# ayildiri/polymer-chemprop

Measured on AMD Instinct MI355X. Metric: edges/sec MPN forward, batch=64 polymer graphs, depth=3 hidden=300, higher is better.
Workload: dtype fp32; 1 GPU; MPNEncoder.forward on synthetic polymer batches of 64 graphs (avg E=6164 directed edges), depth=3, hidden=300, 8 resident batches cycled per rank; global_batch=64, depth=3, hidden=300, parallelism=dp1 (independent graphs, no collective in the forward), streams=3

## Files before the change

### polymer-chemprop_amd/csrc/fused_mp.hpp

```cpp
#pragma once
#include "gemm_x6.hpp"
#include "kernels.hpp"
#include "wdmpnn.h"

namespace wd {


constexpr int BLK_BONDS = 128, BLK_ATOMS = 64;
constexpr int BLK_MOLS = 64;
constexpr int ELLW = 8;
static_assert(ELLW % 4 == 0, "ELL rows of whole 4-byte index words and float4 weight groups");

struct EllRow {
    uint32_t ix[ELLW / 4];
    float w[ELLW];
};
__device__ __forceinline__ EllRow ell_zero() {
    EllRow e;
    for (int k = 0; k < ELLW / 4; ++k) e.ix[k] = 0;
    for (int k = 0; k < ELLW; ++k) e.w[k] = 0.f;
    return e;
}
__device__ __forceinline__ EllRow ell_load(const uint8_t *idx, const float *coef, size_t row) {
    EllRow e;
// ... 52 lines not shown
    const uint8_t *ain; int ain_g;
    uint8_t *aout;
    uint8_t *apairs;
};

template <int BM, int AACT>
struct H2Prod {
    static constexpr int U = BM / 64;
    static constexpr int SETS = 3;
    __amdgpu_buffer_rsrc_t rs;
    int off[U];
    uint32_t grow[U];
    int r0, u, live16;
    float slope, scale, pd;
    uint64_t seed;
    uint32_t layer;
    uint32_t wv;
    u32x4 v[SETS][U][2];
    __device__ __forceinline__ void init() { scale = h2_scale(wave_max_u32(wv)); }
    __device__ __forceinline__ H2Prod(const MpLayerP &P, int rs0, int rn, uint32_t words) {
        const int t = threadIdx.x & 255;
        r0 = t >> 2; u = t & 3;
        rs = __builtin_amdgcn_make_buffer_rsrc(const_cast<float *>(P.zin + (size_t)rs0 * P.ldz), 0,
                                               rn > 0 ? ((rn - 1) * P.ldz + P.kp) * 4 : 0, 0x00020000);
#pragma unroll
        for (int i = 0; i < U; ++i) {
            const int r = r0 + 64 * i;
            grow[i] = r < rn ? rs0 + r : 0;
            off[i] = (r * P.ldz + 8 * u) * 4;
        }
        live16 = (rn + 15) & ~15;
        slope = AACT == ACT_PRELU ? P.slope[0] : 0.f;
        wv = words;
        scale = 1.f;
        pd = P.p_drop_in;
        seed = P.seed;
        layer = P.layer - 1;
    }
    template <typename S>
    __device__ __forceinline__ void load(S, int kc) {
#pragma unroll
        for (int i = 0; i < U; ++i)
#pragma unroll
            for (int h = 0; h < 2; ++h)
                v[S::value][i][h] = __builtin_bit_cast(u32x4, __builtin_amdgcn_raw_buffer_load_b128(rs, off[i] + 128 * kc + 16 * h, 0, 0));
    }
    template <typename S>
    __device__ __forceinline__ void store(S, int kc, uint8_t *st) {
#pragma unroll
        for (int i = 0; i < U; ++i)
#pragma unroll
            for (int h = 0; h < 2; ++h) asm volatile("" ::"v"(v[S::value][i][h]));
#pragma unroll
        for (int i = 0; i < U; ++i) {
            const int r = r0 + 64 * i;
            if (r >= live16) continue;
            float x[8];
#pragma unroll
            for (int h = 0; h < 2; ++h) {
                const u32x4 a = v[S::value][i][h];
                x[4 * h] = __uint_as_float(a.x); x[4 * h + 1] = __uint_as_float(a.y);
                x[4 * h + 2] = __uint_as_float(a.z); x[4 * h + 3] = __uint_as_float(a.w);
            }
#pragma unroll
            for (int q = 0; q < 8; ++q) x[q] = act_fwd(AACT, x[q], slope);
            if (pd > 0.f)
#pragma unroll
                for (int q = 0; q < 8; ++q) x[q] *= dropout_scale(seed, layer, grow[i], 32 * kc + 8 * u + q, pd);
            uint32_t hh[4], ll[4];
#pragma unroll
            for (int q = 0; q < 4; ++q) split_h2(x[2 * q], x[2 * q + 1], scale, hh[q], ll[q]);
            uint8_t *d = st + x6_slot(r, u);
            *reinterpret_cast<u32x4 *>(d) = u32x4{hh[0], hh[1], hh[2], hh[3]};
            *reinterpret_cast<u32x4 *>(d + BM * 64) = u32x4{ll[0], ll[1], ll[2], ll[3]};
        }
    }
};

#ifndef WD_ZWT
#define WD_ZWT 0
#endif

constexpr int MP_THREADS = 512;

template <int BN, int NT, bool LAST, bool ATOM = false, bool POUT = false>
struct MpEpilogue {
    static constexpr int BM = BLK_BONDS, LDC = BN + 4;
    static constexpr int UPR = BN / 8, UNITS = BM * UPR, UPT = (UNITS + NT - 1) / NT;
    static constexpr int AUNITS = BLK_ATOMS * UPR, AUPT = (AUNITS + NT - 1) / NT;
    static constexpr int LDS_FLOATS = (BM + BLK_ATOMS) * LDC;
    static constexpr int YPT = ATOM ? AUPT : UPT;
    EllRow aell[AUPT];
    EllRow gell[ATOM && LAST ? AUPT : 1];
    int32_t rv[ATOM ? 1 : UPT];
    uint32_t sa[ATOM ? 1 : UPT];

    __device__ __forceinline__ void prefetch(const MpLayerP &P, const BlockRow &B) {
        const int tid = threadIdx.x;
#pragma unroll
        for (int i = 0; i < AUPT; ++i) {
            const int v = tid + NT * i;
            const bool ok = v < AUNITS && v / UPR < B.an;
            aell[i] = ell_zero();
            if (ok) aell[i] = ATOM ? ell_load(P.mell_idx, P.mell_coef, (size_t)B.as + v / UPR)
                                   : ell_load(P.aell_idx, P.aell_coef, (size_t)B.as + v / UPR);
            if constexpr (ATOM && LAST) {
                gell[i] = ell_zero();
                if (ok) gell[i] = ell_load(P.aell_idx, P.aell_coef, (size_t)B.as + v / UPR);
            }
        }
        if constexpr (!ATOM)
#pragma unroll
            for (int i = 0; i < UPT; ++i) {
                const int v = tid + NT * i, lr = v / UPR;
                rv[i] = 0;
                sa[i] = 0;
                if (v < UNITS && lr < B.bn) {
                    rv[i] = P.rev[B.bs + lr];
                    sa[i] = P.src_blk[B.bs + lr];
                }
            }
    }

    static constexpr int PRE_ELL = BLK_ATOMS * (int)sizeof(EllRow);
    static constexpr int PRE_BYTES = PRE_ELL * (ATOM && LAST ? 2 : 1) + (ATOM ? 0 : BM * 8);
    __device__ __forceinline__ void fill_pre(const MpLayerP &P, const BlockRow &B, uint8_t *pre) {
        const int t = threadIdx.x - MP_THREADS / 2;
        if (t < BLK_ATOMS) {
            EllRow e = ell_zero();
            if (t < B.an) e = ATOM ? ell_load(P.mell_idx, P.mell_coef, (size_t)B.as + t)
                                   : ell_load(P.aell_idx, P.aell_coef, (size_t)B.as + t);
            reinterpret_cast<EllRow *>(pre)[t] = e;
            if constexpr (ATOM && LAST) {
                EllRow f = ell_zero();
                if (t < B.an) f = ell_load(P.aell_idx, P.aell_coef, (size_t)B.as + t);
                reinterpret_cast<EllRow *>(pre + PRE_ELL)[t] = f;
            }
        }
        if constexpr (!ATOM)
            if (t < BM) {
                int2 q = make_int2(0, 0);
                if (t < B.bn) q = make_int2(P.rev[B.bs + t], (int)P.src_blk[B.bs + t]);
                reinterpret_cast<int2 *>(pre + PRE_ELL)[t] = q;
            }
    }
    __device__ __forceinline__ void take_pre(const BlockRow &B, const uint8_t *pre) {
        const int tid = threadIdx.x;
#pragma unroll
        for (int i = 0; i < AUPT; ++i) {
            const int v = tid + NT * i, la = min(v / UPR, BLK_ATOMS - 1);
            aell[i] = reinterpret_cast<const EllRow *>(pre)[la];
            if constexpr (ATOM && LAST) gell[i] = reinterpret_cast<const EllRow *>(pre + PRE_ELL)[la];
        }
        if constexpr (!ATOM)
#pragma unroll
            for (int i = 0; i < UPT; ++i) {
                const int v = tid + NT * i, lr = min(v / UPR, BM - 1);
                const int2 q = reinterpret_cast<const int2 *>(pre + PRE_ELL)[lr];
                rv[i] = q.x;
                sa[i] = (uint32_t)q.y;
            }
    }

    __device__ __forceinline__ void row_sum(const int32_t *ptr, const int32_t *idx, const float *coef, int row, int base,
                                            const EllRow &E, int c, const float *T, float4 &s0, float4 &s1) {
        s0 = s1 = f4zero();
#pragma unroll
        for (int k = 0; k < ELLW; ++k)
            if (E.w[k] != 0.f) lds_term<LDC>(T, ell_idx(E, k), c, E.w[k], s0, s1);
        if (ell_more(E))
            for (int q = ptr[row] + ELLW; q < ptr[row + 1]; ++q) {
                const int li = idx[q] - base;
                if (li >= 0) lds_term<LDC>(T, li, c, coef ? coef[q] : 1.0f, s0, s1);
            }
    }
    __device__ __forceinline__ void atom_sum(const MpLayerP &P, const BlockRow &B, const EllRow &E, int la, int c,
                                             const float *T, float4 &s0, float4 &s1) {
        row_sum(P.aptr, P.aidx, P.acoef, B.as + la, ATOM ? B.as : B.bs, E, c, T, s0, s1);
    }

    template <int ACT>
    __device__ __forceinline__ void run(const MpLayerP &P, const BlockRow &B, int blk, int n0, float *Pt) {
        const int tid = threadIdx.x;
        float *At = Pt + BM * LDC;
        const int rs = ATOM ? B.as : B.bs, rn = ATOM ? B.an : B.bn;
        constexpr int NU = ATOM ? AUNITS : UNITS, PT = ATOM ? AUPT : UPT;
        float4 res[PT][2];
#pragma unroll
        for (int i = 0; i < PT; ++i) {
            const int v = tid + NT * i, lr = v / UPR, c = 8 * (v % UPR);
            res[i][0] = res[i][1] = f4zero();
            if (v < NU && lr < rn) {
                const float *s = P.inp + (size_t)(rs + lr) * P.ldr + n0 + c;
                res[i][0] = ld4(s);
                res[i][1] = ld4(s + 4);
            }
        }
        if constexpr (!ATOM) {
            if (P.undirected) {
#pragma unroll
                for (int i = 0; i < UPT; ++i) {
                    const int v = tid + NT * i, lr = v / UPR, c = 8 * (v % UPR);
                    const int rl = rv[i] - B.bs;
                    if (v < UNITS && lr < B.bn && lr < rl) {
                        float4 p0 = ld4(Pt + lr * LDC + c), p1 = ld4(Pt + lr * LDC + c + 4);
                        const float4 q0 = ld4(Pt + rl * LDC + c), q1 = ld4(Pt + rl * LDC + c + 4);
                        p0.x = (p0.x + q0.x) / 2.0f; p0.y = (p0.y + q0.y) / 2.0f;
                        p0.z = (p0.z + q0.z) / 2.0f; p0.w = (p0.w + q0.w) / 2.0f;
                        p1.x = (p1.x + q1.x) / 2.0f; p1.y = (p1.y + q1.y) / 2.0f;
                        p1.z = (p1.z + q1.z) / 2.0f; p1.w = (p1.w + q1.w) / 2.0f;
                        st4(Pt + lr * LDC + c, p0); st4(Pt + lr * LDC + c + 4, p1);
                        st4(Pt + rl * LDC + c, p0); st4(Pt + rl * LDC + c + 4, p1);
                    }
                }
                __syncthreads();
            }
            wd_stamp(4 + 8 * LAST);
#pragma unroll
            for (int i = 0; i < AUPT; ++i) {
                const int v = tid + NT * i, la = v / UPR, c = 8 * (v % UPR);
                if (v >= AUNITS || la >= B.an) break;
                float4 s0, s1;
                atom_sum(P, B, aell[i], la, c, Pt, s0, s1);
                st4(At + la * LDC + c, s0);
                st4(At + la * LDC + c + 4, s1);
            }
            __syncthreads();
// ... 61 lines not shown
            const __amdgpu_buffer_rsrc_t prs = __builtin_amdgcn_make_buffer_rsrc(
                P.aout + (size_t)blk * (P.kp >> 5) * CH, 0, (P.kp >> 5) * CH, 0x00020000);
#pragma unroll
            for (int i = 0; i < PT; ++i) {
                const int v = tid + NT * i, lr = v / UPR, c = 8 * (v % UPR);
                if (v >= NU || lr >= ((rn + 15) & ~15)) break;
                h2_store8(prs, h2_blk_off<BM>(lr, n0 + c), BM * 64, ym[i][0], ym[i][1], s);
            }
        } else if constexpr (!LAST) {
            __shared__ uint32_t red[MP_THREADS / 64];
            publish_max(mx, P.amax_out + (size_t)blk * P.n_tiles + n0 / BN, red);
        }
        if constexpr (LAST) {
            __syncthreads();
            float *Mt = Pt;
#pragma unroll
            for (int i = 0; i < PT; ++i) {
                const int v = tid + NT * i, lr = v / UPR, c = 8 * (v % UPR);
                if (v >= NU) break;
                st4(Mt + lr * LDC + c, ym[i][0]);
                st4(Mt + lr * LDC + c + 4, ym[i][1]);
            }
            __syncthreads();
            if (POUT && P.apairs) {
                float4 as[AUPT][2];
                uint32_t amx = 0;
#pragma unroll
                for (int i = 0; i < AUPT; ++i) {
                    const int v = tid + NT * i, la = v / UPR, c = 8 * (v % UPR);
                    as[i][0] = as[i][1] = f4zero();
                    if (v < AUNITS && la < B.an) {
                        atom_sum(P, B, aell[i], la, c, Mt, as[i][0], as[i][1]);
                        const float q[8] = {as[i][0].x, as[i][0].y, as[i][0].z, as[i][0].w,
                                            as[i][1].x, as[i][1].y, as[i][1].z, as[i][1].w};
#pragma unroll
                        for (int k = 0; k < 8; ++k) amx = max(amx, absbits(q[k]));
                    }
                }
                __shared__ uint32_t red[MP_THREADS / 64];
                const float s = h2_scale(publish_max_all(amx, P.amax_out + (size_t)blk * P.n_tiles + n0 / BN, red));
                constexpr int CHA = 2 * BLK_ATOMS * 64;
                const __amdgpu_buffer_rsrc_t prs = __builtin_amdgcn_make_buffer_rsrc(
                    P.apairs + (size_t)blk * (P.kp >> 5) * CHA, 0, (P.kp >> 5) * CHA, 0x00020000);
#pragma unroll
                for (int i = 0; i < AUPT; ++i) {
                    const int v = tid + NT * i, la = v / UPR, c = 8 * (v % UPR);
                    if (v >= AUNITS || la >= ((B.an + 15) & ~15)) break;
                    h2_store8(prs, h2_blk_off<BLK_ATOMS>(la, n0 + c), BLK_ATOMS * 64, as[i][0], as[i][1], s);
                }
            } else {
            const __amdgpu_buffer_rsrc_t ars = x6_block_rsrc<BLK_ATOMS>(P.aplanes, P.kp, blk);
#pragma unroll
            for (int i = 0; i < AUPT; ++i) {
                const int v = tid + NT * i, la = v / UPR, c = 8 * (v % UPR);
                if (v >= AUNITS || la >= B.an) break;
                float4 s0, s1;
                if constexpr (ATOM) atom_sum(P, B, gell[i], la, c, Mt, s0, s1);
                else atom_sum(P, B, aell[i], la, c, Mt, s0, s1);
                x6_store8_blk<BLK_ATOMS>(ars, la, n0 + c, s0, s1);
                if (P.asave) {
                    float *ar = P.asave + (size_t)(B.as + la) * P.kp + n0 + c;
                    st4(ar, s0);
                    st4(ar + 4, s1);
                }
            }
            }
        }
    }
};

template <int BN, bool LAST, int ACT, bool ATOM = false, int NJ = WD_MULTI, bool PAIRS = false>
__global__ __launch_bounds__(MP_THREADS, 4) void mp_layer_kernel(const Multi<MpLayerP, NJ> MP) {
    constexpr int BM = BLK_BONDS;
    using Epi_ = MpEpilogue<BN, MP_THREADS, LAST, ATOM, PAIRS>;
    constexpr int EPI_BYTES = Epi_::LDS_FLOATS * 4;
    constexpr int STG_BYTES = PAIRS ? h2p_lds_bytes<BM, BN>() : h2_lds_bytes<BM, BN>();
    constexpr int LDS_BYTES = EPI_BYTES > STG_BYTES ? EPI_BYTES : STG_BYTES;
    static_assert(LDS_BYTES <= (PAIRS && H2P_STAGES > 3 ? 160 : 80) * 1024, "two workgroups per CU");
    __shared__ __attribute__((aligned(16))) uint8_t lds[LDS_BYTES];
    int tile;
    wd_stamp(0 + 8 * LAST);
    const MpLayerP &P = multi_pick(MP, xcd_tile(blockIdx.x, gridDim.x), tile);
    const int blk = tile / P.n_tiles, nt = tile % P.n_tiles, n0 = nt * BN;
    const BlockRow B = load_block(P.blocks, blk);
    Epi_ E;
    float *Pt = reinterpret_cast<float *>(lds);
    const int rs = ATOM ? B.as : B.bs, rn = ATOM ? B.an : B.bn;
    if constexpr (PAIRS) {
        static_assert(!ATOM, "pair operands: bond messages");
        static_assert(EPI_BYTES + Epi_::PRE_BYTES <= STG_BYTES, "epilogue lists beside the P tile");
        uint8_t *pre = lds + STG_BYTES - Epi_::PRE_BYTES;
        const uint32_t wv = lane_word(P.amax_in + (size_t)blk * P.amax_in_n, P.amax_in_n);
        const uint32_t whm = *P.wh_amax;
        wd_stamp(1 + 8 * LAST);
        floatx4 acc[BM / 64][BN / 16];
        int se;
        constexpr int CH = 2 * BM * 64;
        h2_mainloop_pairs<BM, BN>(P.ain + (size_t)blk * (P.kp >> 5) * CH, P.wh + (size_t)nt * (P.kp >> 5) * (2 * BN * 64),
                                  P.kp >> 5, rn, wv, P.ain_g, lds, acc, se);
        wd_stamp(2 + 8 * LAST);
        if (threadIdx.x >= MP_THREADS / 2) E.fill_pre(P, B, pre);
        __syncthreads();
        E.take_pre(B, pre);
        wd_stamp(3 + 8 * LAST);
        if (threadIdx.x < 256) {
            const float ia = se >= 0 ? __uint_as_float((uint32_t)(254 - se) << 23) : 1.f;
            x6_acc_to_lds_scaled<BM, BN, 4, 1>(acc, Pt, ia, h2_inv_scale(whm));
        }
        __syncthreads();
        E.template run<ACT>(P, B, blk, n0, Pt);
        wd_stamp(6 + 8 * LAST);
        if (blk == 0 && threadIdx.x < BN / 4) {
            float *zr = LAST ? P.zsave : P.zout;
            if (zr) st4(zr + n0 + 4 * threadIdx.x, f4zero());
            if (LAST && P.asave) st4(P.asave + n0 + 4 * threadIdx.x, f4zero());
        }
    } else {
    int w0 = blk * P.amax_in_n, wn = P.amax_in_n;
    if (P.amax_rt > 0) {
        const int t0 = rs / P.amax_rt, t1 = (rs + max(rn, 1) - 1) / P.amax_rt;
        w0 = t0 * P.amax_in_n;
        wn = (t1 - t0 + 1) * P.amax_in_n;
    }
    const uint32_t wv = lane_word(P.amax_in + w0, wn);
    const uint32_t whm = *P.wh_amax;
    H2Prod<BM, ACT> ap(P, rs, rn, wv);
    wd_stamp(1 + 8 * LAST);
    floatx4 acc[BM / 64][BN / 16];
    h2_mainloop_ws<BM, BN>(P.wh + (size_t)nt * (P.kp >> 5) * (2 * BN * 64), P.kp >> 5, rn, lds, acc, ap);
    wd_stamp(2 + 8 * LAST);
#ifndef WD_EPI_PRE
#define WD_EPI_PRE 1
#endif
    __shared__ __attribute__((aligned(16))) uint8_t pre[WD_EPI_PRE ? Epi_::PRE_BYTES : 16];
    static_assert(LDS_BYTES + (WD_EPI_PRE ? Epi_::PRE_BYTES : 0) + 64 <= 80 * 1024, "two workgroups per CU");
    if (WD_EPI_PRE) {
        if (threadIdx.x >= MP_THREADS / 2) E.fill_pre(P, B, pre);
    } else {
        E.prefetch(P, B);
    }
    __syncthreads();
    if (WD_EPI_PRE) E.take_pre(B, pre);
    wd_stamp(3 + 8 * LAST);
    const float ia = h2_inv_scale(wave_max_u32(wv));
    const float iw = h2_inv_scale(whm);
    if (threadIdx.x < 256) x6_acc_to_lds_scaled<BM, BN, 4, 1>(acc, Pt, ia, iw);
    __syncthreads();
    E.template run<ACT>(P, B, blk, n0, Pt);
    wd_stamp(6 + 8 * LAST);
    if (blk == 0 && threadIdx.x < BN / 4) {
        float *zr = LAST ? P.zsave : P.zout;
        if (zr) st4(zr + n0 + 4 * threadIdx.x, f4zero());
        if (LAST && P.asave) st4(P.asave + n0 + 4 * threadIdx.x, f4zero());
    }
    }
}

struct EmbedP {
    const WdAtomCode *codes;
    const uint8_t *src_blk;
    const uint16_t *tail;
    const float *wt;
    const float *woat;
    float *eo;
    const float *bias;
    const int32_t *blocks;
    int Fa, Fb, Hk, n_tiles;
    float *inp;
    const float *slope;
    uint32_t *amax;
    uint8_t *m0;
};

template <int LDT>
__device__ __forceinline__ float4 code_sum(const WdAtomCode &cd, const float *T, int Fa, int c) {
    float4 s = f4zero();
#pragma unroll
    for (int q = 0; q < 8; ++q) {
        if (cd.col[q] == 0xFF) continue;
        const float4 w = ld4(T + cd.col[q] * LDT + c);
        s.x += w.x; s.y += w.y; s.z += w.z; s.w += w.w;
    }
    fma4(s, cd.last, ld4(T + (Fa - 1) * LDT + c));
    return s;
}

#ifndef WD_EMBED_EO_LAST
#define WD_EMBED_EO_LAST 0
#endif
template <int BN, int ACT, int NJ = WD_MULTI, bool PAIRS = false>
__global__ __launch_bounds__(512) void embed_kernel(const Multi<EmbedP, NJ> MP) {
    constexpr bool EO_LAST = WD_EMBED_EO_LAST;
    static_assert(!PAIRS || BN % 16 == 0, "pair groups of whole 16-column halves");
    constexpr int NT = 512, LDC = BN + 4, C4 = BN / 4, U8 = BN / 8, MAXK = 160, PER = (MAXK * C4 + NT - 1) / NT;
    constexpr int BU = (BLK_BONDS * U8 + NT - 1) / NT;
    __shared__ __attribute__((aligned(16))) float wt[MAXK * BN];
    __shared__ __attribute__((aligned(16))) float ea[BLK_ATOMS * LDC];
    __shared__ __attribute__((aligned(16))) float bb[BN];
    __shared__ WdAtomCode code[BLK_ATOMS];
    static_assert(sizeof(float) * (MAXK * BN + BLK_ATOMS * LDC + BN) + sizeof(WdAtomCode) * BLK_ATOMS <= 80 * 1024,
// ... 74 lines not shown
            const float4 w0 = ld4(w), w1 = ld4(w + 4);
            z0.x += w0.x; z0.y += w0.y; z0.z += w0.z; z0.w += w0.w;
            z1.x += w1.x; z1.y += w1.y; z1.z += w1.z; z1.w += w1.w;
        }
        const float4 b0 = ld4(bb + c), b1 = ld4(bb + c + 4);
        z0.x += b0.x; z0.y += b0.y; z0.z += b0.z; z0.w += b0.w;
        z1.x += b1.x; z1.y += b1.y; z1.z += b1.z; z1.w += b1.w;
        float *zr = P.inp + (size_t)b * P.Hk + n0 + c;
        st4(zr, z0);
        st4(zr + 4, z1);
        float zz[8] = {z0.x, z0.y, z0.z, z0.w, z1.x, z1.y, z1.z, z1.w};
#pragma unroll
        for (int q = 0; q < 8; ++q) {
            zz[q] = act_fwd(ACT, zz[q], slope);
            mx = max(mx, absbits(zz[q]));
        }
        if constexpr (PAIRS) {
            ym[u][0] = make_float4(zz[0], zz[1], zz[2], zz[3]);
            ym[u][1] = make_float4(zz[4], zz[5], zz[6], zz[7]);
        }
    }
    if (blk == 0 && tid < C4) st4(P.inp + n0 + 4 * tid, f4zero());
    wd_estamp(5);
    __shared__ uint32_t red[NT / 64];
    if constexpr (PAIRS) {
        const float s = h2_scale(publish_max_all(mx, P.amax + (size_t)blk * P.n_tiles + nt, red));
        wd_estamp(6);
        constexpr int CH = 2 * BLK_BONDS * 64;
        const __amdgpu_buffer_rsrc_t prs = __builtin_amdgcn_make_buffer_rsrc(
            P.m0 + (size_t)blk * (P.Hk >> 5) * CH, 0, (P.Hk >> 5) * CH, 0x00020000);
#pragma unroll
        for (int u = 0; u < BU; ++u) {
            const int v = tid + NT * u, lb = v / U8, c = 8 * (v % U8);
            if (lb >= ((B.bn + 15) & ~15)) break;
            h2_store8(prs, h2_blk_off<BLK_BONDS>(lb, n0 + c), BLK_BONDS * 64, ym[u][0], ym[u][1], s);
        }
        wd_estamp(7);
    } else {
        publish_max(mx, P.amax + (size_t)blk * P.n_tiles + nt, red);
    }
    if constexpr (EO_LAST) {
        __syncthreads();
        eo_half();
    }
}

constexpr int WO_MAXK = 160;

struct WoReadoutP {
    const uint8_t *fa; int kpa; int kca;
    int kcw;
    const uint8_t *ag; int kp;
    const uint8_t *wo;
    const float *bias;
    const int32_t *blocks;
    const float *w_atoms; const int32_t *mol_start, *mol_size; const float *xn;
    int agg; float norm; const float *zero_vec;
    int act; const float *slope; float p_drop; uint64_t seed; uint32_t layer;
    float *out; int ncols;
    int n_tiles;
    const float *eo;
    int Hk, ldeo;
    float *zosave;
    const uint8_t *apairs; const uint32_t *a_amax; int a_nw, a_g;
    const uint8_t *woh; const uint32_t *wo_amax;
};

template <int BN> struct WoWaves;
template <> struct WoWaves<64> { static constexpr int WM = 4, WN = 2; };
template <> struct WoWaves<80> { static constexpr int WM = 2, WN = 5; };

template <int BN, int CPS, int NJ = WD_MULTI, bool PAIRS = false>
__global__ __launch_bounds__(PAIRS ? 512 : 64 * WoWaves<BN>::WM * WoWaves<BN>::WN, PAIRS ? 4 : 1) void wo_readout_kernel(const Multi<WoReadoutP, NJ> MP) {
    constexpr int BM = BLK_ATOMS, LDC = BN + 4, WM = PAIRS ? 4 : WoWaves<BN>::WM, WN = PAIRS ? 1 : WoWaves<BN>::WN;
    constexpr int NT = PAIRS ? 512 : 64 * WM * WN;
    constexpr int WS = 2;
    constexpr int EPI_BYTES = (BM * LDC + BM + 3 * BLK_MOLS + BN) * 4;
    constexpr int LDS_BYTES = PAIRS ? (h2p_lds_bytes<BM, BN>() > EPI_BYTES ? h2p_lds_bytes<BM, BN>() : EPI_BYTES)
                                    : WS * CPS * x6_stage_bytes<BM, BN>();
    __shared__ __attribute__((aligned(16))) uint8_t lds[LDS_BYTES];
    int tile;
    const WoReadoutP &P = multi_pick(MP, xcd_tile(blockIdx.x, gridDim.x), tile);
    const int blk = tile / P.n_tiles, nt = tile % P.n_tiles, n0 = nt * BN;
    const BlockRow B = load_block(P.blocks, blk);
    const int tid = threadIdx.x;
    X6Operands O{};
    O.a0 = P.fa; O.nkc0 = P.kpa >> 5; O.kc0 = P.kca;
    O.a1 = P.ag; O.nkc1 = P.kp >> 5; O.kc1 = P.kp >> 5;
    O.rb = blk;
    O.a_rows = B.an;
    O.b = P.wo + ((size_t)nt * (P.kcw + (P.kp >> 5)) + (P.kcw - P.kca)) * (3 * BN * 64);
    constexpr int C4 = BN / 4;
    static_assert((PAIRS || NT % C4 == 0) && BM <= NT, "one bias group per thread, one atom weight per thread");
    const int nm = min(B.mh - B.ml, BLK_MOLS);
    if (P.zosave && blk == 0 && tid < BN / 4) st4(P.zosave + n0 + 4 * tid, f4zero());
    float4 bb = f4zero();
    float watom = 0.f, mxn = 0.f;
    int mstart = 0, msize = 0;
    constexpr int EPU = (BM * C4 + NT - 1) / NT;
    float4 eo[EPU];
    auto prefetch = [&](int phase) {
        if (phase != 0) return;
        if (!PAIRS || tid < C4) bb = ld4(P.bias + n0 + 4 * (tid % C4));
        if (tid < B.an) watom = P.w_atoms[B.as + tid];
#pragma unroll
        for (int j = 0; j < EPU; ++j) {
            const int v = tid + NT * j, la = v / C4, c = 4 * (v % C4);
            eo[j] = P.eo && v < BM * C4 && la < B.an ? ld4(P.eo + (size_t)(B.as + la) * P.ldeo + n0 + c) : f4zero();
        }
        if (tid < nm) {
            mstart = P.mol_start[B.ml + tid];
            msize = P.mol_size[B.ml + tid];
            mxn = P.xn[B.ml + tid];
        }
    };
    float *H = reinterpret_cast<float *>(lds);
    floatx4 acc[BM / WM / 16][BN / WN / 16];
    if constexpr (PAIRS) {
        prefetch(0);
        const uint32_t wv = threadIdx.x < 256 ? lane_word(P.a_amax + (size_t)blk * P.a_nw, P.a_nw) : 0u;
        int se;
        h2_mainloop_pairs<BM, BN>(P.apairs + (size_t)blk * (P.kp >> 5) * (2 * BM * 64),
                                  P.woh + (size_t)nt * (P.kp >> 5) * (2 * BN * 64), P.kp >> 5, B.an, wv, P.a_g, lds,
                                  acc, se);
        __syncthreads();
        if (threadIdx.x < 256)
            x6_acc_to_lds_scaled<BM, BN, 4, 1>(acc, H, se >= 0 ? __uint_as_float((uint32_t)(254 - se) << 23) : 1.f,
                                               h2_inv_scale(*P.wo_amax));
    } else {
        x6_mainloop<BM, BN, WM, WN, WS, CPS>(O, lds, acc, prefetch);
        __syncthreads();
        x6_acc_to_lds<BM, BN, WM, WN>(acc, H);
    }
    float *Wl = H + BM * LDC;
    float *Ml = Wl + BM;
    static_assert(EPI_BYTES <= LDS_BYTES, "readout staging fits");
    static_assert(BLK_MOLS <= NT, "one molecule per thread in the prefetch");
    if (tid < BM) Wl[tid] = watom;
    if (PAIRS && tid < C4) st4(Ml + 3 * BLK_MOLS + 4 * tid, bb);
    if (tid < nm) {
        Ml[tid] = __int_as_float(mstart);
        Ml[BLK_MOLS + tid] = __int_as_float(msize);
        Ml[2 * BLK_MOLS + tid] = mxn;
    }
    __syncthreads();
    with_act(P.act, [&](auto act_c) {
        constexpr int ACT = decltype(act_c)::value;
        const float slope = ACT == ACT_PRELU ? P.slope[0] : 0.f;
#pragma unroll
        for (int j = 0; j < EPU; ++j) {
            const int v = tid + NT * j;
            if (v >= BM * C4) break;
            const int la = v / C4, c = 4 * (v % C4);
            float4 hv = ld4(H + la * LDC + c);
            hv.x += eo[j].x; hv.y += eo[j].y; hv.z += eo[j].z; hv.w += eo[j].w;
            const float4 b4 = PAIRS ? ld4(Ml + 3 * BLK_MOLS + c) : bb;
            float z[4] = {hv.x + b4.x, hv.y + b4.y, hv.z + b4.z, hv.w + b4.w};
            if (P.zosave && la < B.an) st4(P.zosave + (size_t)(B.as + la) * P.Hk + n0 + c, make_float4(z[0], z[1], z[2], z[3]));
#pragma unroll
            for (int q = 0; q < 4; ++q) z[q] = act_fwd(ACT, z[q], slope);
            if (P.p_drop > 0.f && la < B.an)
#pragma unroll
                for (int q = 0; q < 4; ++q) z[q] *= dropout_scale(P.seed, P.layer, B.as + la, n0 + c + q, P.p_drop);
            st4(H + la * LDC + c, make_float4(z[0], z[1], z[2], z[3]));
        }
    });
    __syncthreads();
    constexpr int RP = 8;
    static_assert(NT % RP == 0 && 64 % RP == 0, "lane groups stay inside a wave");
    for (int t = tid; t < nm * BN * RP; t += NT) {
        const int part = t % RP, u = t / RP, im = u / BN, i = B.ml + im, cc = u % BN, col = n0 + cc;
        const int n = __float_as_int(Ml[BLK_MOLS + im]);
        float s = 0.f, wsum = 0.f;
        const int a0 = __float_as_int(Ml[im]) - B.as;
        for (int a = part; a < n; a += RP) {
            const float w = Wl[a0 + a];
            s = fmaf(w, H[(a0 + a) * LDC + cc], s);
            wsum += w;
        }
#pragma unroll
        for (int off = 1; off < RP; off <<= 1) {
            s += __shfl_xor(s, off, 64);
            wsum += __shfl_xor(wsum, off, 64);
        }
        if (part != 0 || col >= P.ncols) continue;
        float v;
        if (n == 0) {
            v = P.zero_vec[col];
        } else {
            const float m = P.agg == 0 ? s / wsum : (P.agg == 2 ? s / P.norm : s);
            v = Ml[2 * BLK_MOLS + im] * m;
        }
        P.out[(size_t)i * P.ncols + col] = v;
    }
}

}
```

### polymer-chemprop_amd/csrc/gemm_x6.hpp

```cpp
#pragma once
#include "gemm.hpp"
#include "planes.hpp"

#include <type_traits>

namespace wd {

#ifndef WD_STAMP_GEMM
#define WD_STAMP_GEMM 0
#endif

struct X6Params {
    const float *a0; int lda0; int ka0;
    const float *a1; int lda1; int ka1;
    const float *bf; int ldb;
    int M, N;
    int tiles_m, tiles_n;
    Epi epi;
    const uint32_t *a_words; int a_cv;
    const uint32_t *b_word;
};

template <int BM, int BK, bool H2 = false>
__global__ __launch_bounds__(4 * BM) void gemm_x6_kernel(X6Params P) {
// ... 736 lines not shown
        const int q = 64 * (4 * j + w4) + lane, p = (q / (BN * 4)) % 2, r = (q >> 2) % BN, sl = q & 3;
        bsrc[j] = p * BPL + r * 64 + 16 * (sl ^ ((r >> 1) & 3));
    }
    auto issue_b = [&](int kc) {
        const uint8_t *bblk = bsrc_base + (size_t)kc * (2 * BPL);
        uint8_t *st = lds + NA * ASTAGE + (kc % NB) * BSTAGE;
#pragma unroll
        for (int j = 0; j < BPW; ++j)
            if (BP % 4 == 0 || 4 * j + w4 < BP) glds16_untracked(bblk + bsrc[j], st + 1024 * (4 * j + w4));
    };
    int ao[TM], bo[TN];
#pragma unroll
    for (int a = 0; a < TM; ++a) ao[a] = x6_slot(32 * w4 + 16 * a + i16, g);
#pragma unroll
    for (int b = 0; b < TN; ++b) bo[b] = x6_slot(16 * b + i16, g);
    const int na = min(TM, max(0, (a_rows - 32 * w4 + 15) >> 4));
    auto compute_n = [&](const uint8_t *st, const uint8_t *sb, auto na_c) {
        constexpr int NA = decltype(na_c)::value;
        f16x8 af[TM][2], bq[2][2];
#pragma unroll
        for (int p = 0; p < 2; ++p) {
#pragma unroll
            for (int a = 0; a < NA; ++a) af[a][p] = *reinterpret_cast<const f16x8 *>(st + p * APL + ao[a]);
            bq[0][p] = *reinterpret_cast<const f16x8 *>(sb + p * BPL + bo[0]);
        }
#pragma unroll
        for (int b = 0; b < TN; ++b) {
#pragma unroll
            for (int a = 0; a < NA; ++a)
                acc[a][b] = __builtin_amdgcn_mfma_f32_16x16x32_f16(af[a][0], bq[b & 1][0], acc[a][b], 0, 0, 0);
            __builtin_amdgcn_sched_barrier(0);
            if (b + 1 < TN)
#pragma unroll
                for (int p = 0; p < 2; ++p) bq[(b + 1) & 1][p] = *reinterpret_cast<const f16x8 *>(sb + p * BPL + bo[b + 1]);
            __builtin_amdgcn_sched_barrier(0);
#pragma unroll
            for (int a = 0; a < NA; ++a) {
                acc[a][b] = __builtin_amdgcn_mfma_f32_16x16x32_f16(af[a][0], bq[b & 1][1], acc[a][b], 0, 0, 0);
                acc[a][b] = __builtin_amdgcn_mfma_f32_16x16x32_f16(af[a][1], bq[b & 1][0], acc[a][b], 0, 0, 0);
            }
            __builtin_amdgcn_sched_barrier(0);
        }
    };
#pragma unroll
    for (int a = 0; a < TM; ++a)
#pragma unroll
        for (int b = 0; b < TN; ++b) acc[a][b] = floatx4{0.f, 0.f, 0.f, 0.f};
    int mine = 0;
#pragma unroll
    for (int j = 0; j < BPW; ++j) mine += BP % 4 == 0 || 4 * j + w4 < BP;
#pragma unroll
    for (int c = 0; c < H2_B_AHEAD; ++c)
        if (c < nchunks) issue_b(c);
    for (int kc = 0; kc < nchunks; ++kc) {
        if (WD_STAMPS && wave == 0) wd_lstamp(kc, 0);
        wait_vmcnt(min(H2_B_AHEAD - 1, nchunks - 1 - kc) * mine);
        asm volatile("s_waitcnt lgkmcnt(0)" ::: "memory");
        if (WD_STAMPS && wave == 0) wd_lstamp(kc, 1);
        __builtin_amdgcn_s_barrier();
        if (WD_STAMPS && wave == 0) wd_lstamp(kc, 2);
        if (kc + H2_B_AHEAD < nchunks) issue_b(kc + H2_B_AHEAD);
        const uint8_t *st = lds + (kc % NA) * ASTAGE, *sb = lds + NA * ASTAGE + (kc % NB) * BSTAGE;
        dispatch_upto<TM>(na, [&](auto c) { compute_n(st, sb, c); });
        if (WD_STAMPS && wave == 0) {
            asm volatile("s_waitcnt lgkmcnt(0)" ::: "memory");
            wd_lstamp(kc, 3);
        }
    }
    __builtin_amdgcn_s_waitcnt(0x0070);
}

#ifndef WD_H2P_STAGES
#define WD_H2P_STAGES 3
#endif
constexpr int H2P_STAGES = WD_H2P_STAGES;
template <int BM, int BN>
constexpr int h2p_stage_bytes() { return 2 * BM * 64 + 2 * BN * 64; }
template <int BM, int BN>
constexpr int h2p_lds_bytes() { return H2P_STAGES * h2p_stage_bytes<BM, BN>(); }

#ifndef WD_H2P_FRAG
#define WD_H2P_FRAG 0
#endif
template <int BM, int BN, int FRAG = WD_H2P_FRAG>
__device__ __forceinline__ void h2_mainloop_pairs(const uint8_t *a_src, const uint8_t *b_src, int nchunks, int a_rows,
                                                  uint32_t wv, int G, uint8_t *lds, floatx4 (&acc)[BM / 64][BN / 16],
                                                  int &se_out) {
    static_assert(BM == 128 || BM == 64, "four consumer waves of BM / 4 rows");
    constexpr int RW = BM / 4, TM = RW / 16, TN = BN / 16;
    constexpr int APL = BM * 64, BPL = BN * 64, STAGE = h2p_stage_bytes<BM, BN>(), NS = H2P_STAGES;
    constexpr int AP = 2 * BM / 16, APW = AP / 4;
    constexpr int BP = 2 * BN / 16, BPW = (BP + 3) / 4;
    static_assert(AP % 4 == 0, "A pieces split evenly over the loader waves");
    const int tid = threadIdx.x, lane = tid & 63, wave = tid >> 6, w4 = wave & 3, g = lane >> 4, i16 = lane & 15;
    const int roff = (NS - (nchunks - 1) % NS) % NS;
#pragma unroll
    for (int a = 0; a < TM; ++a)
#pragma unroll
        for (int b = 0; b < TN; ++b) acc[a][b] = floatx4{0.f, 0.f, 0.f, 0.f};
    if (wave >= 4) {
        int src[APW + BPW], dst[APW + BPW];
        bool on[APW + BPW];
        int mine = 0;
#pragma unroll
        for (int j = 0; j < APW; ++j) {
            const int c = 4 * j + w4, q = 64 * c + lane, p = q / (BM * 4), r = (q >> 2) % BM, sl = q & 3;
            src[j] = p * APL + r * 64 + 16 * (sl ^ ((r >> 1) & 3));
            dst[j] = 1024 * c;
            on[j] = 16 * (c % (BM / 16)) < a_rows;
            mine += on[j];
        }
#pragma unroll
        for (int j = 0; j < BPW; ++j) {
            const int c = 4 * j + w4, q = 64 * c + lane, p = (q / (BN * 4)) % 2, r = (q >> 2) % BN, sl = q & 3;
            src[APW + j] = p * BPL + r * 64 + 16 * (sl ^ ((r >> 1) & 3));
            dst[APW + j] = 2 * APL + 1024 * c;
            on[APW + j] = BP % 4 == 0 || c < BP;
            mine += on[APW + j];
        }
        mine = __builtin_amdgcn_readfirstlane(mine);
        auto issue = [&](int kc) {
            uint8_t *st = lds + ((kc + roff) % NS) * STAGE;
            const uint8_t *ablk = a_src + (size_t)kc * (2 * APL), *bblk = b_src + (size_t)kc * (2 * BPL);
#pragma unroll
            for (int j = 0; j < APW; ++j)
                if (on[j]) glds16_untracked(ablk + src[j], st + dst[j]);
#pragma unroll
            for (int j = 0; j < BPW; ++j)
                if (on[APW + j]) glds16_untracked(bblk + src[APW + j], st + dst[APW + j]);
        };
#pragma unroll
        for (int c = 0; c < NS - 1; ++c)
            if (c < nchunks) issue(c);
        dispatch_upto<APW + BPW>(mine, [&](auto m_c) {
            constexpr int M = decltype(m_c)::value;
            for (int kc = 0; kc < nchunks; ++kc) {
                if (WD_STAMPS && wave == 4) wd_lstamp(kc, 4);
                if (nchunks - 1 - kc >= NS - 2) asm volatile("s_waitcnt vmcnt(%0)" ::"n"((NS - 2) * M) : "memory");
                else wait_vmcnt((nchunks - 1 - kc) * M);
                if (WD_STAMPS && wave == 4) wd_lstamp(kc, 5);
                __builtin_amdgcn_s_barrier();
                if (kc + NS - 1 < nchunks) issue(kc + NS - 1);
            }
        });
        __builtin_amdgcn_s_waitcnt(0x0070);
        se_out = -1;
        return;
    }
    int ao[TM], bo[TN];
#pragma unroll
    for (int a = 0; a < TM; ++a) ao[a] = x6_slot(RW * w4 + 16 * a + i16, g);
#pragma unroll
    for (int b = 0; b < TN; ++b) bo[b] = x6_slot(16 * b + i16, g);
    const int na = min(TM, max(0, (a_rows - RW * w4 + 15) >> 4));
    constexpr int BIG = 1 << 20;
    const int k0 = min((32 * lane) / G, 63), k1 = min((32 * lane + 16) / G, 63);
    const uint32_t lw0 = (uint32_t)__shfl((int)wv, k0, 64), lw1 = (uint32_t)__shfl((int)wv, k1, 64);
    const int s0 = lw0 ? h2_sexp(lw0) : BIG, s1 = lw1 ? h2_sexp(lw1) : BIG;
    const int cur = BIG - (int)wave_max_u32((uint32_t)(BIG - (lane < nchunks ? min(s0, s1) : BIG)));
    auto f16code = [&](int se) -> uint32_t {
        const int d = se - cur;
        return d > 24 ? 0u : (uint32_t)__builtin_bit_cast(unsigned short, (_Float16)__builtin_amdgcn_ldexpf(1.0f, -d));
    };
    const uint32_t fcode = f16code(s0) | (f16code(s1) << 16);
    const int fsh = lane < 32 ? 0 : 16;
    auto compute_n = [&](const uint8_t *st, const uint8_t *sb, auto na_c, _Float16 fl) {
        constexpr int NA = decltype(na_c)::value;
        constexpr int SCH = FRAG & 3, NB = SCH == 2 ? TN : 2;
        f16x8 af[TM][2], bq[NB][2];
#pragma unroll
        for (int p = 0; p < 2; ++p) {
#pragma unroll
            for (int a = 0; a < NA; ++a) {
                af[a][p] = *reinterpret_cast<const f16x8 *>(st + p * APL + ao[a]);
                af[a][p] = af[a][p] * fl;
            }
#pragma unroll
            for (int b = 0; b < (SCH == 2 ? TN : 1); ++b) bq[b][p] = *reinterpret_cast<const f16x8 *>(sb + p * BPL + bo[b]);
        }
#pragma unroll
        for (int b = 0; b < TN; ++b) {
            const int cb = SCH == 2 ? b : (b & 1);
            if constexpr (SCH == 1) {
                if (b + 1 < TN)
#pragma unroll
                    for (int p = 0; p < 2; ++p) bq[(b + 1) & 1][p] = *reinterpret_cast<const f16x8 *>(sb + p * BPL + bo[b + 1]);
                __builtin_amdgcn_sched_barrier(0);
            }
#pragma unroll
            for (int a = 0; a < NA; ++a)
                acc[a][b] = __builtin_amdgcn_mfma_f32_16x16x32_f16(af[a][0], bq[cb][0], acc[a][b], 0, 0, 0);
            __builtin_amdgcn_sched_barrier(0);
            if (SCH == 0 && b + 1 < TN)
#pragma unroll
                for (int p = 0; p < 2; ++p) bq[(b + 1) & 1][p] = *reinterpret_cast<const f16x8 *>(sb + p * BPL + bo[b + 1]);
            __builtin_amdgcn_sched_barrier(0);
#pragma unroll
            for (int a = 0; a < NA; ++a) {
                acc[a][b] = __builtin_amdgcn_mfma_f32_16x16x32_f16(af[a][0], bq[cb][1], acc[a][b], 0, 0, 0);
                acc[a][b] = __builtin_amdgcn_mfma_f32_16x16x32_f16(af[a][1], bq[cb][0], acc[a][b], 0, 0, 0);
            }
            __builtin_amdgcn_sched_barrier(0);
        }
    };
    dispatch_upto<TM>(na, [&](auto na_c) {
        for (int kc = 0; kc < nchunks; ++kc) {
            if (WD_STAMPS && wave == 0) wd_lstamp(kc, 0);
            asm volatile("s_waitcnt lgkmcnt(0)" ::: "memory");
            if (WD_STAMPS && wave == 0) wd_lstamp(kc, 1);
            __builtin_amdgcn_s_barrier();
            if (WD_STAMPS && wave == 0) wd_lstamp(kc, 2);
            const uint8_t *st = lds + ((kc + roff) % NS) * STAGE, *sb = st + 2 * APL;
            const uint32_t fc = __builtin_amdgcn_readlane(fcode, kc);
            const _Float16 fl = __builtin_bit_cast(_Float16, (unsigned short)((fc >> fsh) & 0xffffu));
            compute_n(st, sb, na_c, fl);
            if (WD_STAMPS && wave == 0) {
                asm volatile("s_waitcnt lgkmcnt(0)" ::: "memory");
                wd_lstamp(kc, 3);
            }
        }
    });
    asm volatile("s_waitcnt lgkmcnt(0)" ::: "memory");
    se_out = cur >= BIG ? -1 : cur;
}

template <int BM, int BN, int WM, int WN>
__device__ __forceinline__ void x6_acc_to_lds(const floatx4 (&acc)[BM / WM / 16][BN / WN / 16], float *cl) {
    constexpr int TM = BM / WM / 16, TN = BN / WN / 16, LDC = BN + 4;
    const int lane = threadIdx.x & 63, wave = threadIdx.x >> 6;
    const int wi = wave / WN, wj = wave % WN, g = lane >> 4, i16 = lane & 15;
#pragma unroll
// ... 62 lines not shown
```

Measured before the change: 241.9 million edges/s.

## Defer block-row and amax loads into pair mainloop and move epilogue list loads to loader waves

The pair GEMM mainloop now takes lazy callbacks for the block row count and the amax scale words. Loader waves fetch block metadata only right before issuing their prologue copies, and consumer waves read the scale words just before computing, so these scalar loads no longer delay the kernel start. The epilogue index and ELL list loads move into a loader hook that runs inside the mainloop on the loader waves, replacing the separate fill step after it. The wave index is made wave-uniform with readfirstlane. Optional early-issue modes sit behind macros that default off. The aim is to hide metadata latency behind the pipelined copies, at the cost of extra register state in the loader waves.

Measured after the change: 247.9 million edges/s, median of 6. +2.5%, better.

```diff
diff --git a/polymer-chemprop_amd/csrc/fused_mp.hpp b/polymer-chemprop_amd/csrc/fused_mp.hpp
--- a/polymer-chemprop_amd/csrc/fused_mp.hpp
+++ b/polymer-chemprop_amd/csrc/fused_mp.hpp
@@ -158,6 +158,9 @@
 #endif
 
 constexpr int MP_THREADS = 512;
+#ifndef WD_PRE_EARLY
+#define WD_PRE_EARLY 0
+#endif
 
 template <int BN, int NT, bool LAST, bool ATOM = false, bool POUT = false>
 struct MpEpilogue {
@@ -200,25 +203,37 @@
 
     static constexpr int PRE_ELL = BLK_ATOMS * (int)sizeof(EllRow);
     static constexpr int PRE_BYTES = PRE_ELL * (ATOM && LAST ? 2 : 1) + (ATOM ? 0 : BM * 8);
-    __device__ __forceinline__ void fill_pre(const MpLayerP &P, const BlockRow &B, uint8_t *pre) {
+    struct Pre {
+        EllRow e, f;
+        int2 q;
+    };
+    __device__ __forceinline__ void load_pre(const MpLayerP &P, const BlockRow &B, Pre &R) {
+        const int t = threadIdx.x - MP_THREADS / 2;
+        R.e = ell_zero();
+        if (t < B.an) R.e = ATOM ? ell_load(P.mell_idx, P.mell_coef, (size_t)B.as + t)
+                                 : ell_load(P.aell_idx, P.aell_coef, (size_t)B.as + t);
+        if constexpr (ATOM && LAST) {
+            R.f = ell_zero();
+            if (t < B.an) R.f = ell_load(P.aell_idx, P.aell_coef, (size_t)B.as + t);
+        }
+        if constexpr (!ATOM) {
+            R.q = make_int2(0, 0);
+            if (t < B.bn) R.q = make_int2(P.rev[B.bs + t], (int)P.src_blk[B.bs + t]);
+        }
+    }
+    __device__ __forceinline__ void store_pre(const Pre &R, uint8_t *pre) {
         const int t = threadIdx.x - MP_THREADS / 2;
         if (t < BLK_ATOMS) {
-            EllRow e = ell_zero();
-            if (t < B.an) e = ATOM ? ell_load(P.mell_idx, P.mell_coef, (size_t)B.as + t)
-                                   : ell_load(P.aell_idx, P.aell_coef, (size_t)B.as + t);
-            reinterpret_cast<EllRow *>(pre)[t] = e;
-            if constexpr (ATOM && LAST) {
-                EllRow f = ell_zero();
-                if (t < B.an) f = ell_load(P.aell_idx, P.aell_coef, (size_t)B.as + t);
-                reinterpret_cast<EllRow *>(pre + PRE_ELL)[t] = f;
-            }
+            reinterpret_cast<EllRow *>(pre)[t] = R.e;
+            if constexpr (ATOM && LAST) reinterpret_cast<EllRow *>(pre + PRE_ELL)[t] = R.f;
         }
         if constexpr (!ATOM)
-            if (t < BM) {
-                int2 q = make_int2(0, 0);
-                if (t < B.bn) q = make_int2(P.rev[B.bs + t], (int)P.src_blk[B.bs + t]);
-                reinterpret_cast<int2 *>(pre + PRE_ELL)[t] = q;
-            }
+            if (t < BM) reinterpret_cast<int2 *>(pre + PRE_ELL)[t] = R.q;
+    }
+    __device__ __forceinline__ void fill_pre(const MpLayerP &P, const BlockRow &B, uint8_t *pre) {
+        Pre R;
+        load_pre(P, B, R);
+        store_pre(R, pre);
     }
     __device__ __forceinline__ void take_pre(const BlockRow &B, const uint8_t *pre) {
         const int tid = threadIdx.x;
@@ -446,24 +461,38 @@
     wd_stamp(0 + 8 * LAST);
     const MpLayerP &P = multi_pick(MP, xcd_tile(blockIdx.x, gridDim.x), tile);
     const int blk = tile / P.n_tiles, nt = tile % P.n_tiles, n0 = nt * BN;
-    const BlockRow B = load_block(P.blocks, blk);
+    BlockRow B = PAIRS ? BlockRow{} : load_block(P.blocks, blk);
     Epi_ E;
     float *Pt = reinterpret_cast<float *>(lds);
-    const int rs = ATOM ? B.as : B.bs, rn = ATOM ? B.an : B.bn;
     if constexpr (PAIRS) {
         static_assert(!ATOM, "pair operands: bond messages");
         static_assert(EPI_BYTES + Epi_::PRE_BYTES <= STG_BYTES, "epilogue lists beside the P tile");
         uint8_t *pre = lds + STG_BYTES - Epi_::PRE_BYTES;
-        const uint32_t wv = lane_word(P.amax_in + (size_t)blk * P.amax_in_n, P.amax_in_n);
-        const uint32_t whm = *P.wh_amax;
+        auto rows = [&]() {
+            B = load_block(P.blocks, blk);
+            return B.bn;
+        };
+        uint32_t whm = 0;
+        auto words = [&]() {
+            whm = *P.wh_amax;
+            return lane_word(P.amax_in + (size_t)blk * P.amax_in_n, P.amax_in_n);
+        };
         wd_stamp(1 + 8 * LAST);
         floatx4 acc[BM / 64][BN / 16];
         int se;
         constexpr int CH = 2 * BM * 64;
+        struct PreHook {
+            Epi_ &E; const MpLayerP &P; const BlockRow &B; uint8_t *pre;
+            typename Epi_::Pre R;
+            __device__ __forceinline__ void issue() { if (WD_PRE_EARLY) E.load_pre(P, B, R); }
+            __device__ __forceinline__ void finish() {
+                if (!WD_PRE_EARLY) E.load_pre(P, B, R);
+                E.store_pre(R, pre);
+            }
+        } hook{E, P, B, pre, {}};
         h2_mainloop_pairs<BM, BN>(P.ain + (size_t)blk * (P.kp >> 5) * CH, P.wh + (size_t)nt * (P.kp >> 5) * (2 * BN * 64),
-                                  P.kp >> 5, rn, wv, P.ain_g, lds, acc, se);
+                                  P.kp >> 5, rows, words, P.ain_g, lds, acc, se, hook);
         wd_stamp(2 + 8 * LAST);
-        if (threadIdx.x >= MP_THREADS / 2) E.fill_pre(P, B, pre);
         __syncthreads();
         E.take_pre(B, pre);
         wd_stamp(3 + 8 * LAST);
@@ -480,6 +509,7 @@
             if (LAST && P.asave) st4(P.asave + n0 + 4 * threadIdx.x, f4zero());
         }
     } else {
+    const int rs = ATOM ? B.as : B.bs, rn = ATOM ? B.an : B.bn;
     int w0 = blk * P.amax_in_n, wn = P.amax_in_n;
     if (P.amax_rt > 0) {
         const int t0 = rs / P.amax_rt, t1 = (rs + max(rn, 1) - 1) / P.amax_rt;
@@ -720,7 +750,7 @@
     int tile;
     const WoReadoutP &P = multi_pick(MP, xcd_tile(blockIdx.x, gridDim.x), tile);
     const int blk = tile / P.n_tiles, nt = tile % P.n_tiles, n0 = nt * BN;
-    const BlockRow B = load_block(P.blocks, blk);
+    BlockRow B = PAIRS ? BlockRow{} : load_block(P.blocks, blk);
     const int tid = threadIdx.x;
     X6Operands O{};
     O.a0 = P.fa; O.nkc0 = P.kpa >> 5; O.kc0 = P.kca;
@@ -730,7 +760,7 @@
     O.b = P.wo + ((size_t)nt * (P.kcw + (P.kp >> 5)) + (P.kcw - P.kca)) * (3 * BN * 64);
     constexpr int C4 = BN / 4;
     static_assert((PAIRS || NT % C4 == 0) && BM <= NT, "one bias group per thread, one atom weight per thread");
-    const int nm = min(B.mh - B.ml, BLK_MOLS);
+    int nm = min(B.mh - B.ml, BLK_MOLS);
     if (P.zosave && blk == 0 && tid < BN / 4) st4(P.zosave + n0 + 4 * tid, f4zero());
     float4 bb = f4zero();
     float watom = 0.f, mxn = 0.f;
@@ -755,16 +785,25 @@
     float *H = reinterpret_cast<float *>(lds);
     floatx4 acc[BM / WM / 16][BN / WN / 16];
     if constexpr (PAIRS) {
-        prefetch(0);
-        const uint32_t wv = threadIdx.x < 256 ? lane_word(P.a_amax + (size_t)blk * P.a_nw, P.a_nw) : 0u;
+        auto rows = [&]() {
+            B = load_block(P.blocks, blk);
+            nm = min(B.mh - B.ml, BLK_MOLS);
+            prefetch(0);
+            return B.an;
+        };
+        uint32_t wom = 0;
+        auto words = [&]() {
+            wom = *P.wo_amax;
+            return lane_word(P.a_amax + (size_t)blk * P.a_nw, P.a_nw);
+        };
         int se;
         h2_mainloop_pairs<BM, BN>(P.apairs + (size_t)blk * (P.kp >> 5) * (2 * BM * 64),
-                                  P.woh + (size_t)nt * (P.kp >> 5) * (2 * BN * 64), P.kp >> 5, B.an, wv, P.a_g, lds,
+                                  P.woh + (size_t)nt * (P.kp >> 5) * (2 * BN * 64), P.kp >> 5, rows, words, P.a_g, lds,
                                   acc, se);
         __syncthreads();
         if (threadIdx.x < 256)
             x6_acc_to_lds_scaled<BM, BN, 4, 1>(acc, H, se >= 0 ? __uint_as_float((uint32_t)(254 - se) << 23) : 1.f,
-                                               h2_inv_scale(*P.wo_amax));
+                                               h2_inv_scale(wom));
     } else {
         x6_mainloop<BM, BN, WM, WN, WS, CPS>(O, lds, acc, prefetch);
         __syncthreads();
diff --git a/polymer-chemprop_amd/csrc/gemm_x6.hpp b/polymer-chemprop_amd/csrc/gemm_x6.hpp
--- a/polymer-chemprop_amd/csrc/gemm_x6.hpp
+++ b/polymer-chemprop_amd/csrc/gemm_x6.hpp
@@ -842,17 +842,29 @@
 #ifndef WD_H2P_FRAG
 #define WD_H2P_FRAG 0
 #endif
-template <int BM, int BN, int FRAG = WD_H2P_FRAG>
-__device__ __forceinline__ void h2_mainloop_pairs(const uint8_t *a_src, const uint8_t *b_src, int nchunks, int a_rows,
-                                                  uint32_t wv, int G, uint8_t *lds, floatx4 (&acc)[BM / 64][BN / 16],
-                                                  int &se_out) {
+#ifndef WD_H2P_EARLY
+#define WD_H2P_EARLY 0
+#endif
+#ifndef WD_H2P_UNIFORM
+#define WD_H2P_UNIFORM 1
+#endif
+struct NoLoaderHook {
+    __device__ void issue() {}
+    __device__ void finish() {}
+};
+template <int BM, int BN, int FRAG = WD_H2P_FRAG, typename Rows, typename Words, typename LoaderHook = NoLoaderHook>
+__device__ __forceinline__ void h2_mainloop_pairs(const uint8_t *a_src, const uint8_t *b_src, int nchunks, Rows &&rows,
+                                                  Words &&words, int G, uint8_t *lds, floatx4 (&acc)[BM / 64][BN / 16],
+                                                  int &se_out, LoaderHook &&lhook = LoaderHook()) {
+    constexpr bool EARLY = WD_H2P_EARLY;
     static_assert(BM == 128 || BM == 64, "four consumer waves of BM / 4 rows");
     constexpr int RW = BM / 4, TM = RW / 16, TN = BN / 16;
     constexpr int APL = BM * 64, BPL = BN * 64, STAGE = h2p_stage_bytes<BM, BN>(), NS = H2P_STAGES;
     constexpr int AP = 2 * BM / 16, APW = AP / 4;
     constexpr int BP = 2 * BN / 16, BPW = (BP + 3) / 4;
     static_assert(AP % 4 == 0, "A pieces split evenly over the loader waves");
-    const int tid = threadIdx.x, lane = tid & 63, wave = tid >> 6, w4 = wave & 3, g = lane >> 4, i16 = lane & 15;
+    const int tid = threadIdx.x, lane = tid & 63, wave = WD_H2P_UNIFORM ? __builtin_amdgcn_readfirstlane(tid >> 6) : tid >> 6, w4 = wave & 3;
+    const int g = lane >> 4, i16 = lane & 15;
     const int roff = (NS - (nchunks - 1) % NS) % NS;
 #pragma unroll
     for (int a = 0; a < TM; ++a)
@@ -860,26 +872,19 @@
         for (int b = 0; b < TN; ++b) acc[a][b] = floatx4{0.f, 0.f, 0.f, 0.f};
     if (wave >= 4) {
         int src[APW + BPW], dst[APW + BPW];
-        bool on[APW + BPW];
-        int mine = 0;
 #pragma unroll
         for (int j = 0; j < APW; ++j) {
             const int c = 4 * j + w4, q = 64 * c + lane, p = q / (BM * 4), r = (q >> 2) % BM, sl = q & 3;
             src[j] = p * APL + r * 64 + 16 * (sl ^ ((r >> 1) & 3));
             dst[j] = 1024 * c;
-            on[j] = 16 * (c % (BM / 16)) < a_rows;
-            mine += on[j];
         }
 #pragma unroll
         for (int j = 0; j < BPW; ++j) {
             const int c = 4 * j + w4, q = 64 * c + lane, p = (q / (BN * 4)) % 2, r = (q >> 2) % BN, sl = q & 3;
             src[APW + j] = p * BPL + r * 64 + 16 * (sl ^ ((r >> 1) & 3));
             dst[APW + j] = 2 * APL + 1024 * c;
-            on[APW + j] = BP % 4 == 0 || c < BP;
-            mine += on[APW + j];
-        }
-        mine = __builtin_amdgcn_readfirstlane(mine);
-        auto issue = [&](int kc) {
+        }
+        auto issue = [&](int kc, const bool (&on)[APW + BPW]) {
             uint8_t *st = lds + ((kc + roff) % NS) * STAGE;
             const uint8_t *ablk = a_src + (size_t)kc * (2 * APL), *bblk = b_src + (size_t)kc * (2 * BPL);
 #pragma unroll
@@ -889,9 +894,36 @@
             for (int j = 0; j < BPW; ++j)
                 if (on[APW + j]) glds16_untracked(bblk + src[APW + j], st + dst[APW + j]);
         };
-#pragma unroll
-        for (int c = 0; c < NS - 1; ++c)
-            if (c < nchunks) issue(c);
+        bool all[APW + BPW], on[APW + BPW];
+#pragma unroll
+        for (int j = 0; j < APW; ++j) all[j] = true;
+#pragma unroll
+        for (int j = 0; j < BPW; ++j) all[APW + j] = BP % 4 == 0 || 4 * j + w4 < BP;
+        if constexpr (EARLY) {
+#pragma unroll
+            for (int c = 0; c < NS - 1; ++c)
+                if (c < nchunks) issue(c, all);
+            __builtin_amdgcn_sched_barrier(0);
+        }
+        const int a_rows = rows();
+        int mine = 0;
+#pragma unroll
+        for (int j = 0; j < APW; ++j) {
+            on[j] = 16 * ((4 * j + w4) % (BM / 16)) < a_rows;
+            mine += on[j];
+        }
+#pragma unroll
+        for (int j = 0; j < BPW; ++j) {
+            on[APW + j] = all[APW + j];
+            mine += on[APW + j];
+        }
+        mine = __builtin_amdgcn_readfirstlane(mine);
+        if constexpr (!EARLY) {
+#pragma unroll
+            for (int c = 0; c < NS - 1; ++c)
+                if (c < nchunks) issue(c, on);
+        }
+        lhook.issue();
         dispatch_upto<APW + BPW>(mine, [&](auto m_c) {
             constexpr int M = decltype(m_c)::value;
             for (int kc = 0; kc < nchunks; ++kc) {
@@ -900,13 +932,16 @@
                 else wait_vmcnt((nchunks - 1 - kc) * M);
                 if (WD_STAMPS && wave == 4) wd_lstamp(kc, 5);
                 __builtin_amdgcn_s_barrier();
-                if (kc + NS - 1 < nchunks) issue(kc + NS - 1);
+                if (kc + NS - 1 < nchunks) issue(kc + NS - 1, on);
             }
         });
         __builtin_amdgcn_s_waitcnt(0x0070);
+        lhook.finish();
         se_out = -1;
         return;
     }
+    const int a_rows = rows();
+    const uint32_t wv = words();
     int ao[TM], bo[TN];
 #pragma unroll
     for (int a = 0; a < TM; ++a) ao[a] = x6_slot(RW * w4 + 16 * a + i16, g);
```
